# zyt334/AdaFace

Measured on AMD Instinct MI355X. Metric: 512x512 images/sec @ 50 DDIM steps, batch 8, higher is better.
Workload: dtype bf16

## Files before the change

adaface_amd/csrc/af_conv_gemm.hip:

```cpp
#include "af_kernels.h"

#include <cstdlib>
#include <cstring>
#include <mutex>
#include <type_traits>

template <int BM, int BN> struct TileCfg {
  static constexpr int XR = BM / 32, WR = BN / 32;
  static constexpr int WM = BM / 2, WN = BN / 2;
  static constexpr int MI = WM / 32, NI = WN / 32;
  static constexpr int TILE_BYTES = (BM + BN) * 128;
  static constexpr int EPI_LD = BN + 4;
  static constexpr int EPI_BYTES = BM * EPI_LD * 4;
  static constexpr int LDS_BYTES = (2 * TILE_BYTES > EPI_BYTES) ? 2 * TILE_BYTES : EPI_BYTES;
};

__device__ __forceinline__ void lds_dma16(__amdgpu_buffer_rsrc_t rs, char* lds_base, unsigned voffset, unsigned soffset) {
#if defined(__HIP_DEVICE_COMPILE__)
  __builtin_amdgcn_raw_ptr_buffer_load_lds(rs, (__attribute__((address_space(3))) void*)lds_base, 16, voffset, soffset,
                                           0, 0);
#endif
}

__device__ __forceinline__ void tile_coords(int wg, int nwg, int ntm, int ntn, int gm, int& tm, int& tn) {
// ... 525 lines not shown
        if (mok && (lane >> 4) == 0)
          *reinterpret_cast<float2*>(p.ln_stats_out + ((long)(tn * 2 + g) * p.M + m) * 2) = float2{ps, pq};
        continue;
      }
      if (slab) {
        if (m >= p.M) continue;
#pragma unroll
        for (int i = 0; i < NI; ++i) {
          if (i >= nblk) continue;
          *reinterpret_cast<f32x4*>(slab + (long)m * p.N + cbase + i * 16) = acc[i][j];
        }
        continue;
      }
      const bool mok2 = m < p.M;
      Quad<T> rq[NI], bq[NI];
      if (rowb && mok2) {
        const T* rp = rowb + (long)(p.howo_shift >= 0 ? m >> p.howo_shift : m / HoWo) * p.ldrb + cbase;
#pragma unroll
        for (int i = 0; i < NI; ++i) if (i < nblk) bq[i].load(rp + i * 16);
      }
      if (res && mok2) {
        const T* rp = res + (long)m * p.ldr + cbase;
#pragma unroll
        for (int i = 0; i < NI; ++i) if (i < nblk) rq[i].load(rp + i * 16);
      }
#pragma unroll
      for (int i = 0; i < NI; ++i) {
        if (i >= nblk) continue;
        Quad<T> o;
#pragma unroll
        for (int e = 0; e < 4; ++e) {
          float v = acc[i][j][e];
          if (rowb && mok2) v += to_f32<T>(bq[i].e[e]);
          if (res && mok2) v += to_f32<T>(rq[i].e[e]);
          o.e[e] = from_f32<T>(v);
        }
        wput(j, i, o);
      }
    }
    if (!slab) wflush();
    if (p.gn_stats_out && !slab && !geglu) {
      const int mslab = m0 + wq * 64;
      if (mslab < p.M) {
        float s = 0.f, q = 0.f;
        if (lane < HNo / 2) {
#pragma unroll 8
          for (int r = 0; r < 64; ++r) {
            const unsigned w = *reinterpret_cast<const unsigned*>(wtile + r * wpitch + lane * 4);
            const float a = __uint_as_float(w << 16), b = __uint_as_float(w & 0xffff0000u);
            s += a + b;
            q += a * a + b * b;
          }
        }
        float2* scr = reinterpret_cast<float2*>(wtile);
        scr[lane] = float2{s, q};
        const int hpg = p.gn_cpg >> 1, ng = (HNo / 2) / hpg;
        if (lane < ng) {
          float a = 0.f, b = 0.f;
          for (int t = 0; t < hpg; ++t) {
            const float2 v = scr[lane * hpg + t];
            a += v.x;
            b += v.y;
          }
          const int hw = 1 << p.howo_shift;
          const long part = ((long)(mslab >> p.howo_shift) * (hw >> 6) + ((mslab & (hw - 1)) >> 6)) * 32 + (ncol0 + g * HNo) / p.gn_cpg + lane;
          *reinterpret_cast<float2*>(p.gn_stats_out + part * 2) = float2{a, b};
        }
      }
    }
    return;
  }
  constexpr int ITEMS = BN / 32;
  const int nitems = geglu ? ITEMS / 2 : ITEMS;
#pragma unroll 1
  for (int pass = 0; pass < 2; ++pass) {
    if (pass) __syncthreads();
    if ((wq >> 1) == pass) {
      const int rbase = (wq & 1) * 64 + (lane & 15);
      const int nblk = geglu ? NI / 2 : NI;
#pragma unroll
      for (int j = 0; j < MI; ++j)
#pragma unroll
        for (int i = 0; i < NI; ++i)
          if (i < nblk)
            *reinterpret_cast<f32x4*>(et + (rbase + j * 16) * C::EPI_LD + g * HNo + i * 16 + cl) = acc[i][j];
    }
    __syncthreads();
    float v[ITEMS][8];
    int im[ITEMS], in_[ITEMS];
    Quad<T> rq[ITEMS][2], bq[ITEMS][2];
#pragma unroll
    for (int it = 0; it < ITEMS; ++it) {
      const int idx = tid + it * 512;
      const int row = geglu ? idx / (BN / 16) : idx / (BN / 8);
      const int c8 = (idx - row * tpr) * 8;
      const int m = m0 + pass * 128 + row, n = ncol0 + c8;
      const bool ok = it < nitems && m < p.M && n < Nvalid;
      im[it] = ok ? m : -1;
      in_[it] = n;
      if (!ok) continue;
      const float4 a = *reinterpret_cast<const float4*>(et + row * C::EPI_LD + c8);
      const float4 b4 = *reinterpret_cast<const float4*>(et + row * C::EPI_LD + c8 + 4);
      v[it][0] = a.x; v[it][1] = a.y; v[it][2] = a.z; v[it][3] = a.w;
      v[it][4] = b4.x; v[it][5] = b4.y; v[it][6] = b4.z; v[it][7] = b4.w;
      if (slab) continue;
      if (rowb) {
        const T* rp = rowb + (long)(p.howo_shift >= 0 ? m >> p.howo_shift : m / HoWo) * p.ldrb + n;
        bq[it][0].load(rp);
        bq[it][1].load(rp + 4);
      }
      if (res) {
        const T* rp = res + (long)m * p.ldr + n;
        rq[it][0].load(rp);
        rq[it][1].load(rp + 4);
      }
    }
#pragma unroll
    for (int it = 0; it < ITEMS; ++it) {
      const int m = im[it], n = in_[it];
      if (m < 0) continue;
      if (slab) {
        *reinterpret_cast<float4*>(slab + (long)m * p.N + n) = float4{v[it][0], v[it][1], v[it][2], v[it][3]};
        *reinterpret_cast<float4*>(slab + (long)m * p.N + n + 4) = float4{v[it][4], v[it][5], v[it][6], v[it][7]};
        continue;
      }
#pragma unroll
      for (int hq = 0; hq < 2; ++hq) {
        float* vv = v[it] + 4 * hq;
        if (rowb) {
#pragma unroll
          for (int e = 0; e < 4; ++e) vv[e] += to_f32<T>(bq[it][hq].e[e]);
        }
        if (res) {
#pragma unroll
          for (int e = 0; e < 4; ++e) vv[e] += to_f32<T>(rq[it][hq].e[e]);
        }
        Quad<T> o;
#pragma unroll
        for (int e = 0; e < 4; ++e) o.e[e] = from_f32<T>(vv[e]);
        o.store(out + (long)m * p.ldo + n + 4 * hq);
      }
    }
  }
}

template <int N> __device__ __forceinline__ void pp_wait_lgkm() {
  __builtin_amdgcn_sched_barrier(0);
  asm volatile("s_waitcnt lgkmcnt(%0)" ::"n"(N) : "memory");
  __builtin_amdgcn_sched_barrier(0);
}
typedef __attribute__((ext_vector_type(8))) int pp_i32x8;
typedef __attribute__((ext_vector_type(4))) int pp_i32x4;

template <int BN, bool GATHER, int LNMODE = 0, bool FP8 = false, int SCHED = FP8 ? 2 : 0>
__global__ __launch_bounds__(512) void conv_gemm_pp_kernel(const ConvGemmParams p) {
  constexpr bool NS = SCHED >= 1, MG = SCHED == 2;
  static_assert(MG || !FP8, "fp8 operands exist on the merged schedule only");
  using C = PpCfg<BN>;
  typedef bf16 T;
  static_assert(!FP8 || LNMODE == 0, "fp8 operands: plain epilogue only");
  constexpr unsigned XE = FP8 ? 1u : 2u;
  constexpr int NI = C::NI, MI = C::MI, SLOT = C::SLOT, XBYTES = C::XBYTES;
  constexpr int XP0 = MG ? C::XP / 2 : C::XP0;
  constexpr int NX0 = XP0 / 4, NX1 = (C::XP - XP0) / 4;
  constexpr int WP0 = MG ? (C::WP / 8) * 4 : 0;
  constexpr int NW0 = WP0 / 4, NW1 = (C::WP - WP0) / 4;
  constexpr int NP0 = NX0 + NW0, NP1 = NX1 + NW1, NPMAX = NP0 > NP1 ? NP0 : NP1;
  constexpr int NXM = NX0 > NX1 ? NX0 : NX1, NWM = NW0 > NW1 ? NW0 : NW1;
  static_assert(XP0 % 4 == 0 && WP0 % 4 == 0 && NW1 >= 1, "piece split");
  extern __shared__ __attribute__((aligned(1024))) char smem[];

  const int tid = threadIdx.x, lane = tid & 63, wid = __builtin_amdgcn_readfirstlane(tid >> 6);
  const int g = wid >> 2, wq = wid & 3;
  const int ntm = (p.M + 255) / 256, ntn = p.N / BN;
  int tm, tn;
  tile_coords(blockIdx.x, gridDim.x, ntm, ntn, p.group_m, tm, tn);
  const int m0 = tm * 256, n0 = tn * BN;
  const int zk = blockIdx.z;
  const int ph4 = (GATHER && p.phase4) ? (int)blockIdx.y : 0;
  const int pad_y = (GATHER && p.phase4) ? 1 - (ph4 >> 1) : p.pad, pad_x = (GATHER && p.phase4) ? 1 - (ph4 & 1) : p.pad;

  const __amdgpu_buffer_rsrc_t rs_x = __builtin_amdgcn_make_buffer_rsrc(
      const_cast<T*>(reinterpret_cast<const T*>(p.src)), 0, (int)0xFFFFFFF0u, 0x00020000);
  const __amdgpu_buffer_rsrc_t rs_w = __builtin_amdgcn_make_buffer_rsrc(
      const_cast<T*>(reinterpret_cast<const T*>(p.W)), 0, (int)0xFFFFFFF0u, 0x00020000);

  const int KT_all = p.K / (FP8 ? 128 : 64);
  const int kt_per = (KT_all + p.splitk - 1) / p.splitk;
  const int kt_begin = zk * kt_per;
  const int KT = min(KT_all, kt_begin + kt_per) - kt_begin;

  const int srow = lane >> 3;
  const unsigned dchunk = (unsigned)((lane & 7) ^ srow);
  const unsigned lchunk = (FP8 ? (dchunk & 3u) : dchunk) * 16u;
  const int HoWo = p.Ho * p.Wo;
  const unsigned ldcb = (unsigned)p.ldc * XE;
  const bool fast_taps = GATHER && ((p.up == 0 && p.ks * p.ks <= 31 && (p.fast_taps & 1)) || MG);
  unsigned x_off[NXM];
  int x_yx[GATHER ? NXM : 1];
  pp_static_for<0, NXM>([&](auto qc) {
    constexpr int q = decltype(qc)::value;
    const int piece = g == 0 ? wq + 4 * q : XP0 + wq + 4 * q;
    const int m = m0 + piece * 8 + srow;
    const bool ok = m < p.M && (g == 0 ? q < NX0 : q < NX1);
    const int mm = ok ? m : 0;
    int b, oy, ox;
    if (p.howo_shift >= 0 && p.wo_shift >= 0) {
      b = mm >> p.howo_shift;
      const int rem = mm & (HoWo - 1);
      oy = rem >> p.wo_shift;
      ox = rem & (p.Wo - 1);
    } else {
      b = mm / HoWo;
      const int rem = mm - b * HoWo;
      oy = rem / p.Wo;
      ox = rem - oy * p.Wo;
    }
    unsigned off = (unsigned)((long)b * p.src_batch_stride * XE) + lchunk;
    if constexpr (GATHER) {
      const int y0 = oy * p.stride - pad_y, x0 = ox * p.stride - pad_x;
      if (fast_taps) {
        int vy = 0, vx = 0;
        for (int k = 0; k < p.ks; ++k) {
          vy |= ((unsigned)(y0 + k) < (unsigned)p.Hi ? 1 : 0) << (k * p.ks);
          vx |= ((unsigned)(x0 + k) < (unsigned)p.Wi ? 1 : 0) << k;
        }
        int msk = 0;
        for (int k = 0; k < p.ks; ++k) msk |= ((vy >> (k * p.ks)) & 1) ? (vx << (k * p.ks)) : 0;
        x_yx[q] = ok ? msk : 0;
        off += (unsigned)(y0 * p.Ws + x0) * ldcb;
      } else {
        x_yx[q] = ok ? ((y0 << 16) | (x0 & 0xffff)) : (int)0xC0000000;
      }
    } else {
      off += (unsigned)(((oy * p.stride) >> p.up) * p.Ws + ((ox * p.stride) >> p.up)) * ldcb;
      if (!ok) off = 0xFFFFFFFFu;
    }
    x_off[q] = off;
  });
  unsigned w_off[NWM];
#pragma unroll
  for (int q = 0; q < NWM; ++q) {
    const int n = n0 + ((g == 0 ? 0 : WP0) + wq + 4 * q) * 8 + srow;
    w_off[q] = n < p.Wrows ? (unsigned)(((long)ph4 * p.Wrows + n) * p.ldw * XE) + dchunk * 16u : 0xFFFFFFFFu;
  }
  struct KWalk {
    int ky, kx, c0, ktile;
    int u_tap, u_c0;
  };
  KWalk kw;
  kw.ktile = kt_begin;
  kw.u_tap = 0; kw.u_c0 = 0;
  if (p.k_tap_inner) {
    const int taps = p.ks * p.ks;
    const int cc = kt_begin / taps, tap = kt_begin - cc * taps;
    kw.c0 = cc * 64;
    kw.ky = tap / p.ks;
    kw.kx = tap - kw.ky * p.ks;
  } else {
    const int k0 = kt_begin * 64;
    const int tap = k0 / p.Cin;
    kw.c0 = k0 - tap * p.Cin;
    kw.ky = tap / p.ks;
    kw.kx = tap - kw.ky * p.ks;
  }
  const int taps8 = p.ks * p.ks;
  const int adv_q = 2 / taps8, adv_r = 2 - adv_q * taps8;
  if constexpr (FP8) {
    const int u = 2 * kt_begin + (int)(dchunk >> 2);
    const int cc = u / taps8;
    kw.u_tap = u - cc * taps8;
    kw.u_c0 = cc * 64;
  }
  struct StageCtx {
    unsigned c0b, k0b;
    int live;
    int tapbit;
    unsigned delta;
    int u_ok;
    unsigned u_delta;
    int ky, kx, u_tap, u_c0;
  };
  auto x_addr = [&](auto qc, auto ftc, const StageCtx& sc) -> unsigned {
    constexpr int q = decltype(qc)::value;
    constexpr bool FT = decltype(ftc)::value;
    if constexpr (FP8) {
      if constexpr (GATHER) {
        if constexpr (FT) return ((x_yx[q] >> sc.u_tap) & sc.u_ok) ? x_off[q] + sc.u_delta : 0xFFFFFFFFu;
        const int kyl = p.ks == 3 ? (sc.u_tap * 11) >> 5 : 0, kxl = p.ks == 3 ? sc.u_tap - 3 * kyl : 0;
        const int iy = (x_yx[q] >> 16) + kyl, ix = ((x_yx[q] << 16) >> 16) + kxl;
        const bool ok = (unsigned)iy < (unsigned)p.Hi && (unsigned)ix < (unsigned)p.Wi && sc.u_c0 < p.Cin;
        const unsigned pix = (unsigned)((iy >> p.up) * p.Ws + (ix >> p.up));
        return ok ? x_off[q] + pix * ldcb + (unsigned)sc.u_c0 : 0xFFFFFFFFu;
      } else {
        return (sc.u_c0 < p.Cin && x_off[q] != 0xFFFFFFFFu) ? x_off[q] + (unsigned)sc.u_c0 : 0xFFFFFFFFu;
      }
    } else if constexpr (GATHER) {
      if constexpr (FT) return (x_yx[q] & sc.tapbit) ? x_off[q] + sc.delta : 0xFFFFFFFFu;
      const int iy = (x_yx[q] >> 16) + sc.ky, ix = ((x_yx[q] << 16) >> 16) + sc.kx;
      const bool ok = (unsigned)iy < (unsigned)p.Hi && (unsigned)ix < (unsigned)p.Wi;
      const unsigned pix = (unsigned)((iy >> p.up) * p.Ws + (ix >> p.up));
      return ok ? x_off[q] + pix * ldcb : 0xFFFFFFFFu;
    } else {
      return x_off[q];
    }
  };
  auto stage_begin = [&](const KWalk& k) -> StageCtx {
    StageCtx sc;
    sc.tapbit = 0; sc.delta = 0u; sc.u_ok = 0; sc.u_delta = 0u;
    sc.ky = k.ky; sc.kx = k.kx; sc.u_tap = k.u_tap; sc.u_c0 = k.u_c0;
// ... 62 lines not shown
  auto wait_keep1 = [&]() { if (g == 0) pp_wait_vm<NP0>(); else pp_wait_vm<NP1>(); };

  const unsigned lds0 = (unsigned)(__UINTPTR_TYPE__)((__attribute__((address_space(3))) char*)smem);
  const unsigned fch0 = (unsigned)((lane >> 4) ^ (lane & 7)) * 16u;
  const unsigned fch1 = (unsigned)(((lane >> 4) + 4) ^ (lane & 7)) * 16u;
  const unsigned x_base = (unsigned)((wq * 64 + (lane & 15)) * 128);
  const unsigned w_base = (unsigned)(XBYTES + (g * C::HN + (lane & 15)) * 128);

  f32x4 acc[NI][MI];
#pragma unroll
  for (int i = 0; i < NI; ++i)
#pragma unroll
    for (int j = 0; j < MI; ++j) acc[i][j] = f32x4{0.f, 0.f, 0.f, 0.f};
  pp_u32x4 xf[MI][2], wf[NI][2];
#pragma unroll
  for (int i = 0; i < NI; ++i) wf[i][1] = pp_u32x4{0u, 0u, 0u, 0u};
#pragma unroll
  for (int j = 0; j < MI; ++j) xf[j][1] = pp_u32x4{0u, 0u, 0u, 0u};

  auto half = [&](int slot_off, auto rc, auto mc) {
    constexpr int ur = decltype(rc)::value, um = decltype(mc)::value;
    const unsigned b = lds0 + (unsigned)slot_off + (ur ? fch1 : fch0);
    pp_static_for<0, NI * MI>([&](auto nc) {
      constexpr int n = decltype(nc)::value;
      constexpr int i = n / MI, j = n % MI;
      if constexpr (n < NI) wf[n][ur] = pp_lds_read128<n * 2048>(b + w_base);
      else if constexpr (n < NI + MI) xf[n - NI][ur] = pp_lds_read128<(n - NI) * 2048>(b + x_base);
      acc[i][j] = __builtin_amdgcn_mfma_f32_16x16x32_bf16(__builtin_bit_cast(bf16x8, wf[i][um]),
                                                          __builtin_bit_cast(bf16x8, xf[j][um]), acc[i][j], 0, 0, 0);
      if constexpr (n < NI + MI) __builtin_amdgcn_sched_barrier(0);
    });
  };
  std::integral_constant<int, 0> U0;
  std::integral_constant<int, 1> U1;

  const int cl = 4 * (lane >> 4);
  float4 bias_r[NI];
  auto load_bias = [&]() {
#pragma unroll
    for (int i = 0; i < NI; ++i) {
      bias_r[i] = float4{0.f, 0.f, 0.f, 0.f};
      if (p.bias && p.splitk <= 1) bias_r[i] = *reinterpret_cast<const float4*>(p.bias + n0 + g * C::HN + i * 16 + cl);
    }
  };
  if constexpr (!NS) load_bias();

  float4 ln_cs[LNMODE == 1 ? NI : 1];
  float ln_mu[LNMODE == 1 ? MI : 1], ln_rs[LNMODE == 1 ? MI : 1];
  if constexpr (LNMODE == 1) {
#pragma unroll
    for (int i = 0; i < NI; ++i) ln_cs[i] = *reinterpret_cast<const float4*>(p.ln_colsum + n0 + g * C::HN + i * 16 + cl);
#pragma unroll
    for (int j = 0; j < MI; ++j) {
      const int m = m0 + wq * 64 + j * 16 + (lane & 15);
      float2 st = float2{0.f, 0.f};
      if (m < p.M) st = *reinterpret_cast<const float2*>(p.ln_stats + (long)m * 2);
      ln_mu[j] = st.x;
      ln_rs[j] = st.y;
    }
  }

  pp_u32x4 w8[NS ? NI : 1][2], xa8[NS ? MI : 1][2], xb8[NS ? MI : 1][2];
  int wsc8[FP8 ? NI : 1];
  int xsc8 = p.x_scale_e8;
  if constexpr (NS && !FP8) {
#pragma unroll
    for (int i = 0; i < NI; ++i) w8[i][0] = w8[i][1] = pp_u32x4{0u, 0u, 0u, 0u};
#pragma unroll
    for (int j = 0; j < MI; ++j) xa8[j][0] = xa8[j][1] = xb8[j][0] = xb8[j][1] = pp_u32x4{0u, 0u, 0u, 0u};
  }
  if constexpr (FP8) {
    asm volatile("" : "+v"(xsc8));
#pragma unroll
    for (int i = 0; i < NI; ++i) {
      w8[i][0] = w8[i][1] = pp_u32x4{0u, 0u, 0u, 0u};
      wsc8[i] = (int)p.w_scale[n0 + g * C::HN + i * 16 + (lane & 15)];
    }
#pragma unroll
    for (int j = 0; j < MI; ++j) xa8[j][0] = xa8[j][1] = xb8[j][0] = xb8[j][1] = pp_u32x4{0u, 0u, 0u, 0u};
  }
  auto mfma8 = [&](f32x4& c, const pp_u32x4 (&wv)[2], const pp_u32x4 (&xv)[2], int wscale) {
    if constexpr (!FP8) {
      c = __builtin_amdgcn_mfma_f32_16x16x32_bf16(__builtin_bit_cast(bf16x8, wv[0]), __builtin_bit_cast(bf16x8, xv[0]), c, 0, 0, 0);
      c = __builtin_amdgcn_mfma_f32_16x16x32_bf16(__builtin_bit_cast(bf16x8, wv[1]), __builtin_bit_cast(bf16x8, xv[1]), c, 0, 0, 0);
      asm volatile("" : "+v"(c));
      return;
    }
    const pp_i32x8 a = __builtin_shufflevector(__builtin_bit_cast(pp_i32x4, wv[0]), __builtin_bit_cast(pp_i32x4, wv[1]), 0, 1, 2, 3, 4, 5, 6, 7);
    const pp_i32x8 b = __builtin_shufflevector(__builtin_bit_cast(pp_i32x4, xv[0]), __builtin_bit_cast(pp_i32x4, xv[1]), 0, 1, 2, 3, 4, 5, 6, 7);
    c = __builtin_amdgcn_mfma_scale_f32_16x16x128_f8f6f4(a, b, c, 0, 0, 0, wscale, 0, xsc8);
    asm volatile("" : "+v"(c));
  };
  auto wait_block = [&](auto nc, pp_u32x4 (&blk)[2]) {
    constexpr int n = decltype(nc)::value;
    asm volatile("s_waitcnt lgkmcnt(%2)" : "+v"(blk[0]), "+v"(blk[1]) : "n"(n) : "memory");
  };
#ifdef AF_LAB_ABLATE
  const int lab = p.fast_taps >> 4;
#else
  constexpr int lab = 0;
#endif
  auto cphase8 = [&](int slot_off, pp_u32x4 (&xc)[NS ? MI : 1][2], pp_u32x4 (&xp)[NS ? MI : 1][2], auto ftc, int stage_off,
                     const StageCtx& sc) {
    if constexpr (NS) {
      constexpr int NB = NI + MI;
      char* sbase = smem + stage_off;
      const unsigned b0 = lds0 + (unsigned)slot_off + fch0, b1 = lds0 + (unsigned)slot_off + fch1;
      auto rd_block = [&](auto bc) {
        constexpr int bi = decltype(bc)::value;
        if (lab & 2) return;
        if constexpr (bi == 0) {
          w8[0][0] = pp_lds_read128<0>(b0 + w_base);
          w8[0][1] = pp_lds_read128<0>(b1 + w_base);
        } else if constexpr (bi <= MI) {
          xc[bi - 1][0] = pp_lds_read128<(bi - 1) * 2048>(b0 + x_base);
          xc[bi - 1][1] = pp_lds_read128<(bi - 1) * 2048>(b1 + x_base);
        } else {
          w8[bi - MI][0] = pp_lds_read128<(bi - MI) * 2048>(b0 + w_base);
          w8[bi - MI][1] = pp_lds_read128<(bi - MI) * 2048>(b1 + w_base);
        }
      };
      rd_block(std::integral_constant<int, 0>{});
      rd_block(std::integral_constant<int, 1>{});
      __builtin_amdgcn_sched_barrier(0);
      pp_static_for<0, MI * NI>([&](auto mc) {
        constexpr int m = decltype(mc)::value;
        if constexpr (m < MI) {
          if (!(lab & 4)) mfma8(acc[NI - 1][m], w8[NI - 1], xp[m], wsc8[FP8 ? NI - 1 : 0]);
        } else {
          constexpr int i = (m - MI) / MI, j = (m - MI) % MI;
          constexpr int issued = (2 + m) < NB ? (2 + m) : NB;
          constexpr int need = i == 0 ? 1 + j : (j == 0 ? MI + i : -1);
          if constexpr (need >= 0) {
            std::integral_constant<int, 2 * (issued - need - 1)> cnt;
            if constexpr (i == 0) wait_block(cnt, xc[j]); else wait_block(cnt, w8[i]);
            if constexpr (i == 0 && j == 0) wait_block(cnt, w8[0]);
          }
          if (!(lab & 4)) mfma8(acc[i][j], w8[i], xc[j], wsc8[FP8 ? i : 0]);
        }
        if constexpr (2 + m < NB) rd_block(std::integral_constant<int, 2 + m>{});
        if constexpr (MG && m >= MI && (m - MI) / 2 < NPMAX) {
          if (!(lab & 1) && (g == ((m - MI) & 1) || !p.pp_stagger)) {
            if (p.pp_stagger || ((m - MI) & 1) == 0) stage_piece(std::integral_constant<int, (m - MI) / 2>{}, ftc, sbase, sc);
          }
        }
        __builtin_amdgcn_sched_barrier(0);
      });
      static_assert(!MG || MI + 2 * (NPMAX - 1) + 1 < MI * NI, "merged schedule: a staging slot behind an MFMA for every piece");
      pp_wait_lgkm0();
    }
  };

  int rd = 0, w0 = SLOT, w1 = 2 * SLOT;
  if constexpr (MG) {
    stage(0);
    stage(SLOT);
    auto tile = [&](auto& xc, auto& xp) {
      if (g == 0) pp_wait_vm<NP0>(); else pp_wait_vm<NP1>();
      __builtin_amdgcn_s_barrier();
      const StageCtx sc = stage_begin(kw);
      cphase8(rd, xc, xp, std::integral_constant<bool, GATHER>{}, w1, sc);
      kw = kw_next(kw);
      const int tmp = rd; rd = w0; w0 = w1; w1 = tmp;
    };
    for (int t = 0; t + 1 < KT; t += 2) {
      tile(xa8, xb8);
      tile(xb8, xa8);
    }
    if (KT & 1) tile(xa8, xb8);
    pp_wait_vm<0>();
    if (KT & 1) {
#pragma unroll
      for (int j = 0; j < MI; ++j) mfma8(acc[NI - 1][j], w8[NI - 1], xa8[j], wsc8[FP8 ? NI - 1 : 0]);
    } else {
#pragma unroll
      for (int j = 0; j < MI; ++j) mfma8(acc[NI - 1][j], w8[NI - 1], xb8[j], wsc8[FP8 ? NI - 1 : 0]);
    }
    __builtin_amdgcn_s_barrier();
  }
  if constexpr (!MG) {
  stage(0);
  if (g == 1) {
    if (KT > 1) { stage(SLOT); wait_keep1(); } else pp_wait_vm<0>();
  }
  __builtin_amdgcn_s_barrier();
  if (g == 1) __builtin_amdgcn_s_barrier();
  }
  auto dphase = [&](int t) {
    if (g == 0) {
      if (t + 1 < KT) { stage(w0); wait_keep1(); } else pp_wait_vm<0>();
    } else {
      if (t + 2 < KT) stage(w1);
    }
    __builtin_amdgcn_s_barrier();
  };
  auto cend = [&](int t) {
    if (g == 1) { if (t + 2 < KT) wait_keep1(); else pp_wait_vm<0>(); }
    __builtin_amdgcn_s_barrier();
    const int tmp = rd; rd = w0; w0 = w1; w1 = tmp;
  };
  if constexpr (MG) {
  } else if constexpr (NS) {
    auto tile1 = [&](int t, auto& xc, auto& xp) {
      dphase(t);
      __builtin_amdgcn_s_setprio(1);
      cphase8(rd, xc, xp, std::false_type{}, 0, StageCtx{});
      __builtin_amdgcn_s_setprio(0);
      cend(t);
    };
    int t = 0;
    for (; t + 1 < KT; t += 2) {
      tile1(t, xa8, xb8);
      tile1(t + 1, xb8, xa8);
    }
    if (KT & 1) tile1(t, xa8, xb8);
    if (KT & 1) {
#pragma unroll
      for (int j = 0; j < MI; ++j) mfma8(acc[NI - 1][j], w8[NI - 1], xa8[j], wsc8[FP8 ? NI - 1 : 0]);
    } else {
#pragma unroll
      for (int j = 0; j < MI; ++j) mfma8(acc[NI - 1][j], w8[NI - 1], xb8[j], wsc8[FP8 ? NI - 1 : 0]);
    }
  } else {
    for (int t = 0; t < KT; ++t) {
      dphase(t);
      __builtin_amdgcn_s_setprio(1);
      half(rd, U0, U1);
      pp_wait_lgkm0();
      half(rd, U1, U0);
      pp_wait_lgkm0();
      __builtin_amdgcn_s_setprio(0);
      cend(t);
    }
#pragma unroll
    for (int i = 0; i < NI; ++i)
#pragma unroll
      for (int j = 0; j < MI; ++j)
        acc[i][j] = __builtin_amdgcn_mfma_f32_16x16x32_bf16(__builtin_bit_cast(bf16x8, wf[i][1]),
                                                            __builtin_bit_cast(bf16x8, xf[j][1]), acc[i][j], 0, 0, 0);
  }
  if constexpr (!MG) { if (g == 0) __builtin_amdgcn_s_barrier(); }
  if constexpr (NS) load_bias();

  pp_epilogue<BN, LNMODE>(p, acc, bias_r, ln_cs, ln_mu, ln_rs, smem, tid, lane, g, wq, m0, n0, tn, zk);
}

#ifdef AF_LAB_ABLATE
__device__ unsigned long long g_lab_stamps[2048 * 5];
extern "C" int af_lab_stamps(unsigned long long* out, int n) {
  return hipMemcpyFromSymbol(out, HIP_SYMBOL(g_lab_stamps), sizeof(unsigned long long) * (size_t)n) == hipSuccess ? 0 : -1;
}
__device__ __forceinline__ unsigned long long lab_now() {
  unsigned long long t;
  __builtin_amdgcn_sched_barrier(0);
  asm volatile("s_memrealtime %0\n\ts_waitcnt lgkmcnt(0)" : "=s"(t)::"memory");
  __builtin_amdgcn_sched_barrier(0);
  return t;
}
#endif
struct Halo8Cfg {
  static constexpr int BN = 160;
  static constexpr int HPIX = 400, HBUF = HPIX * 128, WBYTES = BN * 128;
  static constexpr int W_BASE = 2 * HBUF, LDS_BYTES = 2 * HBUF + 3 * WBYTES;
  static constexpr int NHQ = 7;
  static_assert(LDS_BYTES <= 160 * 1024, "LDS budget");
};

template <int LABL>
__global__ __launch_bounds__(512) void conv3x3_halo8_kernel(const ConvGemmParams p) {
  using C = PpCfg<160>;
  using H = Halo8Cfg;
  typedef bf16 T;
  constexpr int BN = 160, NI = C::NI, MI = C::MI, NHQ = H::NHQ;
  extern __shared__ __attribute__((aligned(1024))) char smem[];
  const int tid = threadIdx.x, lane = tid & 63, wid = __builtin_amdgcn_readfirstlane(tid >> 6);
  const int g = wid >> 2, wq = wid & 3;
  const int ntm = p.M / 256, ntn = p.N / BN;
  int tm, tn;
  tile_coords(blockIdx.x, gridDim.x, ntm, ntn, p.group_m, tm, tn);
  const int m0 = tm * 256, n0 = tn * BN;
  const int zk = blockIdx.z;
  T* const xsrc = const_cast<T*>(reinterpret_cast<const T*>(p.src));
  T* const wsrc = const_cast<T*>(reinterpret_cast<const T*>(p.W));
  const __amdgpu_buffer_rsrc_t rs_x = __builtin_amdgcn_make_buffer_rsrc(xsrc, 0, (int)0xFFFFFFF0u, 0x00020000);
  const __amdgpu_buffer_rsrc_t rs_w = __builtin_amdgcn_make_buffer_rsrc(wsrc, 0, (int)0xFFFFFFF0u, 0x00020000);

  const int KT_all = p.K / 64;
  const int kt_per = (KT_all + p.splitk - 1) / p.splitk;
  const int kt_begin = zk * kt_per;
#ifdef AF_LAB_ABLATE
  const int lab = p.fast_taps >> 4;
  const int KT = (lab & 16) ? 9 : min(KT_all, kt_begin + kt_per) - kt_begin;
#else
  constexpr int lab = 0;
  const int KT = min(KT_all, kt_begin + kt_per) - kt_begin;
#endif
  const int chunk0 = kt_begin / 9;
  const int nch = KT / 9;
#ifdef AF_LAB_ABLATE
  unsigned long long st0 = 0, st1 = 0, st2 = 0;
  if (lab & 64) st0 = lab_now();
#endif

  const int Wo = p.Wo, HW = Wo + 2, wsh = p.wo_shift;
  const int R = 256 >> wsh;
  const int HP = (R + 2) * HW;
  const int img = m0 >> p.howo_shift;
// ... 1203 lines not shown
  const long nbs = nb * s;
  const double fill = (double)nbs / (double)(((nbs + 255) / 256) * 256);
  if (fill < g_af_knobs.gemm_pp_minfill * 0.01) return pl;
  pl.tile = cand;
  pl.splitk = s;
  if (s > 1) pl.ws_bytes = (size_t)s * p.M * p.N * sizeof(float);
  plan_group_m(pl, p);
  return pl;
}

AfGemmPlan af_plan_conv_gemm(const ConvGemmParams& p, int batch, int elem_size) {
  if (p.fp8) return plan_fp8(p, batch);
  AfGemmPlan pl;
  pl.tile = 0;
  pl.splitk = 1;
  pl.ws_bytes = 0;
  const bool geglu = p.epilogue == AF_EPI_GEGLU;
  const bool n128 = geglu || (p.N % 128) == 0 || p.N > 640;
  static const int bm[4] = {128, 64, 128, 64}, bn[4] = {128, 128, 64, 64};
  static const double eff[4] = {1.0, 0.88, 0.88, 0.72};
  double best = 1e30;
  for (int t = 0; t < 4; ++t) {
    if (n128 && bn[t] != 128) continue;
    if (!n128 && bn[t] != 64) continue;
    const long nb = (long)((p.M + bm[t] - 1) / bm[t]) * ((p.N + bn[t] - 1) / bn[t]) * batch;
    const double rounds = (double)((nb + 255) / 256);
    const double cost = rounds * bm[t] * bn[t] / eff[t];
    if (cost < best) { best = cost; pl.tile = t; }
  }
  const int BK = 128 / elem_size;
  const int KT = p.K / BK;
  const long nb = (long)((p.M + bm[pl.tile] - 1) / bm[pl.tile]) * ((p.N + bn[pl.tile] - 1) / bn[pl.tile]) * batch;
  if (batch == 1 && !geglu && nb < 256 && KT >= 16) {
    const int target = g_af_knobs.splitk_target;
    int s = (int)((target + nb - 1) / nb);
    if (s > KT / 8) s = KT / 8;
    if (s > 16) s = 16;
    if (s >= 2) {
      pl.tile = n128 ? 0 : 2;
      const long nb2 = (long)((p.M + bm[pl.tile] - 1) / bm[pl.tile]) * ((p.N + bn[pl.tile] - 1) / bn[pl.tile]);
      s = (int)((target + nb2 - 1) / nb2);
      if (s > KT / 8) s = KT / 8;
      if (s > 16) s = 16;
      if (s >= 2) pl.splitk = s;
    }
  }
  if (g_af_knobs.small_m_tile64 && batch == 1 && !geglu && p.M <= 1024 && p.N % 64 == 0 && KT <= 32) {
    const long nb64 = (long)((p.M + 63) / 64) * (p.N / 64);
    if (nb64 >= 64 && nb64 <= 1024) { pl.tile = 3; pl.splitk = 1; }
  }
  pl.halo_tw = 0;
  if (p.ks == 3 && p.stride == 1 && p.up == 0 && p.pad == 1 && batch == 1 && !geglu && pl.splitk == 1 &&
      p.Ho == p.Hi && p.Wo == p.Wi && p.ldc >= p.Cin && g_af_knobs.conv_halo) {
    if (p.Wo % 32 == 0 && p.Ho % 4 == 0) pl.halo_tw = 32;
    else if (p.Wo % 16 == 0 && p.Ho % 8 == 0) pl.halo_tw = 16;
    if (pl.halo_tw) {
      const long nb128 = (long)(p.M / 128) * ((p.N + 127) / 128), nb64 = (long)(p.M / 128) * ((p.N + 63) / 64);
      const double c128 = (double)((nb128 + 255) / 256) * 128, c64 = (double)((nb64 + 255) / 256) * 64 / 0.9;
      pl.tile = (n128 && c128 <= c64) ? 0 : 2;
      if (!n128 && (p.N % 64) != 0) pl.tile = 2;
    }
  }
  if (elem_size == 2 && batch == 1 && p.K % 64 == 0 && p.Cin % 64 == 0 && g_af_knobs.gemm_pp) {
    int cand = -1;
    if (!geglu && p.N % 160 == 0) cand = 5;
    else if (p.N % 128 == 0) cand = 4;
    if (cand >= 0) {
      const int tbn = cand == 5 ? 160 : 128;
      const long nb = (long)((p.M + 255) / 256) * (p.N / tbn);
      int s = 1;
      if (!geglu && nb < 208) {
        s = (int)((256 + nb / 2) / nb);
        if (s > KT / 16) s = KT / 16;
        if (s > 16) s = 16;
        if (s < 1) s = 1;
      }
      const long nbs = nb * s;
      const double fill = (double)nbs / (double)(((nbs + 255) / 256) * 256);
      if (fill >= g_af_knobs.gemm_pp_minfill * 0.01 && p.M >= 512) {
        pl.tile = cand;
        pl.splitk = s;
        pl.halo_tw = 0;
      }
    }
  }
  if (pl.tile == 5 && pl.halo_tw == 0 && p.ks == 3 && p.stride == 1 && p.pad == 1 && p.up == 0 && p.Ho == p.Hi && p.Wo == p.Wi &&
      (p.Wo == 16 || p.Wo == 32 || p.Wo == 64) && (p.Ho & (p.Ho - 1)) == 0 && p.Ho >= 256 / p.Wo && p.M % 256 == 0 &&
      p.K == 9 * p.Cin && p.ldc >= p.Cin && (g_af_knobs.conv_halo8 & 1) && !p.ln_stats && !p.ln_stats_out) {
    pl.halo_tw = 256;
    while (pl.splitk > 1 && (p.Cin / 64) % pl.splitk != 0) --pl.splitk;
  }
  if (elem_size == 2 && (g_af_knobs.conv_halo8 & 2) && g_af_knobs.gemm_pp && af_conv_s8_ok(p, batch) && !p.gn_stats_out &&
      (p.Wo <= 16 || (g_af_knobs.conv_halo8 & 4))) {
    pl.tile = 5;
    pl.halo_tw = 8;
    pl.splitk = af_conv_s8_slices(p, batch);
  }
  const int ft = g_af_knobs.gemm_tile;
  if (ft >= 0 && ft < 4 && !(geglu && bn[ft] != 128)) pl.tile = ft;
  const int fs = g_af_knobs.gemm_splitk;
  if (fs >= 1 && batch == 1 && !geglu) pl.splitk = fs > KT ? KT : fs;
  if (pl.halo_tw == 8 && (pl.tile != 5 || pl.splitk != af_conv_s8_slices(p, batch))) pl.halo_tw = 0;
  if (pl.splitk > 1 && pl.halo_tw != 256 && pl.halo_tw != 8) pl.halo_tw = 0;
  if (pl.halo_tw == 256 && (pl.tile != 5 || (p.Cin / 64) % pl.splitk != 0)) pl.halo_tw = 0;
  if (pl.splitk > 1) pl.ws_bytes = (size_t)pl.splitk * p.M * p.N * sizeof(float);
  plan_group_m(pl, p);
  return pl;
}

static void plan_group_m(AfGemmPlan& pl, const ConvGemmParams& p) {
  static const int bm[4] = {128, 64, 128, 64}, bn[4] = {128, 128, 64, 64};
  {
    const bool h4 = pl.halo_tw != 0 && pl.halo_tw != 256 && pl.halo_tw != 8;
    const int tbm = h4 ? 128 : (pl.tile >= 4 ? 256 : bm[pl.tile]);
    const int tbn = h4 ? ((pl.tile == 0 || pl.tile == 1) ? 128 : 64) : (pl.tile == 5 ? 160 : pl.tile == 4 ? 128 : bn[pl.tile]);
    const int MT = (p.M + tbm - 1) / tbm, NT = (p.N + tbn - 1) / tbn;
    const int resident = pl.tile >= 4 ? 32 : 32 * ((tbm * tbn >= 128 * 128) ? 2 : 3);
    const bool taps_reuse = pl.halo_tw || (pl.tile >= 4 && p.ks > 1 && (g_af_knobs.conv_tap_inner || p.fp8));
    const double xb = (double)p.M * (p.K / (p.ks * p.ks)) * (taps_reuse ? (p.stride == 1 ? 1.5 : 1.0) : (double)(p.ks * p.ks) / (p.stride * p.stride));
    const double wb = (double)p.N * p.K;
    double bestc = 1e300;
    int bestg = 1;
    for (int gmm = 1; gmm <= 64; gmm *= 2) {
      const int gm_eff = gmm < MT ? gmm : MT;
      int gn_eff = resident / gm_eff;
      if (gn_eff < 1) gn_eff = 1;
      if (gn_eff > NT) gn_eff = NT;
      const double c = xb * ((double)NT / gn_eff) + wb * ((double)MT / gm_eff);
      if (c < bestc * 0.999) { bestc = c; bestg = gmm; }
    }
    pl.group_m = g_af_knobs.gemm_groupm >= 1 ? g_af_knobs.gemm_groupm : bestg;
  }
}

template <typename T, int BM, int BN, bool DMA>
static int launch_cfg2(const ConvGemmParams& p, int batch, hipStream_t stream) {
  using C = TileCfg<BM, BN>;
  static unsigned long long attr_done = 0;
  if (int rc = af_ensure_dynamic_lds(attr_done, reinterpret_cast<const void*>(&conv_gemm_kernel<T, BM, BN, DMA>), C::LDS_BYTES)) return rc;
  const int ntm = (p.M + BM - 1) / BM, ntn = (p.N + BN - 1) / BN;
  dim3 grid(ntm * ntn, 1, p.splitk > 1 ? p.splitk : batch);
  hipLaunchKernelGGL((conv_gemm_kernel<T, BM, BN, DMA>), grid, dim3(256), C::LDS_BYTES, stream, p);
  HIP_CHECK_RET(hipGetLastError());
  return 0;
}
template <typename T, int BM, int BN>
static int launch_cfg(const ConvGemmParams& p, int batch, hipStream_t stream) {
  const int force = g_af_knobs.gemm_dma;
  const int kt_per_slice = p.K / (128 / (int)sizeof(T)) / (p.splitk > 1 ? p.splitk : 1);
  const bool use_dma = force >= 0 ? force != 0 : kt_per_slice >= 32;
  return use_dma ? launch_cfg2<T, BM, BN, true>(p, batch, stream) : launch_cfg2<T, BM, BN, false>(p, batch, stream);
}

template <int BN, int LNMODE, bool GATHER, bool FP8, int SCHED>
static int launch_pp_one(const ConvGemmParams& p, dim3 grid, hipStream_t stream) {
  using C = PpCfg<BN>;
  static unsigned long long attr_done = 0;
  if (int rc = af_ensure_dynamic_lds(attr_done, reinterpret_cast<const void*>(&conv_gemm_pp_kernel<BN, GATHER, LNMODE, FP8, SCHED>), C::LDS_BYTES)) return rc;
  hipLaunchKernelGGL((conv_gemm_pp_kernel<BN, GATHER, LNMODE, FP8, SCHED>), grid, dim3(512), C::LDS_BYTES, stream, p);
  HIP_CHECK_RET(hipGetLastError());
  return 0;
}
template <int BN, int LNMODE, bool GATHER> static int launch_pp_sched(const ConvGemmParams& p, dim3 grid, hipStream_t stream) {
  int sched = g_af_knobs.pp_sched;
  if (sched >= 2 && GATHER && !(p.up == 0 && p.ks * p.ks <= 31)) sched = 1;
  if (p.epilogue == AF_EPI_GEGLU && g_af_knobs.pp_sched == 2) sched = 0;
  switch (sched) {
    case 0: return launch_pp_one<BN, LNMODE, GATHER, false, 0>(p, grid, stream);
    case 1: return launch_pp_one<BN, LNMODE, GATHER, false, 1>(p, grid, stream);
    default: return launch_pp_one<BN, LNMODE, GATHER, false, 2>(p, grid, stream);
  }
}
template <int BN> static int launch_pp(const ConvGemmParams& p, hipStream_t stream) {
  const bool gather = !(p.ks == 1 && p.pad == 0);
  dim3 grid(((p.M + 255) / 256) * (p.N / BN), 1, p.splitk > 1 ? p.splitk : 1);
  if (p.ln_stats || p.ln_stats_out) {
    if (gather || p.splitk > 1 || (p.ln_stats && p.ln_stats_out) || (p.ln_stats_out && p.epilogue == AF_EPI_GEGLU)) {
      af_set_error_msg("conv_gemm: LayerNorm-fused launch needs a 1x1 GEMM without split-K");
      return -1;
    }
    return p.ln_stats ? launch_pp_sched<BN, 1, false>(p, grid, stream) : launch_pp_sched<BN, 2, false>(p, grid, stream);
  }
  return gather ? launch_pp_sched<BN, 0, true>(p, grid, stream) : launch_pp_sched<BN, 0, false>(p, grid, stream);
}

template <int BN> static int launch_pp8(const ConvGemmParams& p, hipStream_t stream) {
  const bool gather = !(p.ks == 1 && p.pad == 0);
  dim3 grid(((p.M + 255) / 256) * (p.N / BN), 1, p.splitk > 1 ? p.splitk : 1);
  return gather ? launch_pp_one<BN, 0, true, true, 2>(p, grid, stream) : launch_pp_one<BN, 0, false, true, 2>(p, grid, stream);
}

static int launch_conv_gemm_fp8(ConvGemmParams p, hipStream_t stream, const AfGemmPlan* plan, void* ws) {
  if (p.K % 128 != 0 || p.Cin % 64 != 0 || (p.ks != 1 && p.ks != 3) || p.K < p.ks * p.ks * p.Cin || p.ldw < p.K ||
      p.ldw % 16 != 0 || p.ldc % 16 != 0 || p.ldc < p.Cin || !p.w_scale || p.epilogue == AF_EPI_GEGLU || p.ln_stats || p.ln_stats_out) {
    af_set_error_msg("conv_gemm fp8: K=%d Cin=%d ks=%d ldw=%d ldc=%d (need K%%128==0, Cin%%64==0, ks 1|3, 16-byte pitches, row scales)",
                     p.K, p.Cin, p.ks, p.ldw, p.ldc);
    return -1;
  }
  if (p.N % 4 != 0 || p.ldo % 4 != 0 || (p.residual && p.ldr % 4 != 0) || (p.rowbias && p.ldrb % 4 != 0)) {
    af_set_error_msg("conv_gemm fp8: N/ldo/ldr/ldrb must be multiples of 4 (N=%d ldo=%d)", p.N, p.ldo);
    return -1;
  }
  if (p.M <= 0 || p.N <= 0) return 0;
  {
    const int HoWo = p.Ho * p.Wo > 0 ? p.Ho * p.Wo : 1;
    const double nb = (double)((p.M + HoWo - 1) / HoWo);
    if (nb * (double)p.src_batch_stride >= 4294967280.0 || (double)p.Wrows * p.ldw >= 4294967280.0) {
      af_set_error_msg("conv_gemm fp8: operand exceeds the 4 GB range of the 32-bit gather offsets (split the batch)");
      return -1;
    }
  }
  AfGemmPlan pl = plan ? *plan : af_plan_conv_gemm(p, 1, 2);
  if (pl.tile != 4 && pl.tile != 5) {
    af_set_error_msg("conv_gemm fp8: shape M=%d N=%d K=%d has no fp8 plan (ask af_plan_conv_gemm first)", p.M, p.N, p.K);
    return -1;
  }
  if (pl.splitk > 1 && !ws) pl.splitk = 1;
  p.splitk = pl.splitk;
  p.ws = ws;
  af_set_last_plan(pl);
  g_af_plan_counts[10] += 1;
  if (pl.splitk > 1) g_af_plan_counts[7] += 1;
  {
    auto lg2 = [](int v) { int s = 0; while ((1 << s) < v) ++s; return (v > 0 && (1 << s) == v) ? s : -1; };
    p.howo_shift = lg2(p.Ho * p.Wo);
    p.wo_shift = lg2(p.Wo);
  }
  p.group_m = pl.group_m > 0 ? pl.group_m : 1;
  p.pp_epilogue = g_af_knobs.pp_direct < 0 ? 0 : (g_af_knobs.pp_direct ? 2 : 1);
  if (p.gn_stats_out) {
    if (!af_conv_gn_stats_ok(p, pl, p.gn_cpg)) {
      af_set_error_msg("conv_gemm fp8: GroupNorm partial sums asked of a launch that cannot write them");
      return -1;
    }
    p.pp_epilogue = 2;
    g_af_plan_counts[14] += 1;
  }
  p.k_tap_inner = 1;
  p.fast_taps = g_af_knobs.conv_fast_taps;
  p.pp_stagger = g_af_knobs.pp_stagger;
  AfProfScope prof(AF_K_PP_FP8, stream, 2.0 * p.M * (double)p.N * (p.k_logical ? p.k_logical : p.K),
                   (double)p.M * p.Cin + (double)p.N * p.K + (double)p.M * p.N * 2.0);
  const int rc = pl.tile == 4 ? launch_pp8<128>(p, stream) : launch_pp8<160>(p, stream);
  if (rc) return rc;
  if (p.splitk > 1) {
    const long nq = (long)p.M * (p.N >> 2);
    unsigned blocks = (unsigned)((nq + 255) / 256);
    if (blocks > 4096) blocks = 4096;
    hipLaunchKernelGGL((splitk_reduce_kernel<bf16>), dim3(blocks), dim3(256), 0, stream, p);
    HIP_CHECK_RET(hipGetLastError());
  }
  return 0;
}

template <int LABL> static int launch_halo8_lab(const ConvGemmParams& p, hipStream_t stream) {
  static unsigned long long attr_done = 0;
  if (int rc = af_ensure_dynamic_lds(attr_done, reinterpret_cast<const void*>(&conv3x3_halo8_kernel<LABL>), Halo8Cfg::LDS_BYTES))
    return rc;
  dim3 grid((p.M / 256) * (p.N / 160), 1, p.splitk > 1 ? p.splitk : 1);
  hipLaunchKernelGGL(conv3x3_halo8_kernel<LABL>, grid, dim3(512), Halo8Cfg::LDS_BYTES, stream, p);
  HIP_CHECK_RET(hipGetLastError());
  return 0;
}
static int launch_halo8(const ConvGemmParams& p, hipStream_t stream) {
  if (p.Cin % 64 != 0 || (p.Cin / 64) % (p.splitk > 1 ? p.splitk : 1) != 0) {
    af_set_error_msg("conv_gemm: halo kernel needs K slices of whole 64-channel chunks (Cin=%d splitk=%d)", p.Cin, p.splitk);
    return -1;
  }
#ifdef AF_LAB_ABLATE
  switch ((p.fast_taps >> 4) & 7) {
    case 1: return launch_halo8_lab<1>(p, stream);
    case 2: return launch_halo8_lab<2>(p, stream);
    case 3: return launch_halo8_lab<3>(p, stream);
    case 4: return launch_halo8_lab<4>(p, stream);
    case 5: return launch_halo8_lab<5>(p, stream);
    case 6: return launch_halo8_lab<6>(p, stream);
    case 7: return launch_halo8_lab<7>(p, stream);
    default: break;
  }
#endif
  return launch_halo8_lab<0>(p, stream);
}

template <typename T, int TW, int BN> static int launch_halo(const ConvGemmParams& p, hipStream_t stream) {
  using C = HaloCfg<TW, BN>;
  static unsigned long long attr_done = 0;
  if (int rc = af_ensure_dynamic_lds(attr_done, reinterpret_cast<const void*>(&conv3x3_halo_kernel<T, TW, BN>), C::LDS_BYTES)) return rc;
  dim3 grid((p.M / 128) * ((p.N + BN - 1) / BN), 1, 1);
  hipLaunchKernelGGL((conv3x3_halo_kernel<T, TW, BN>), grid, dim3(256), C::LDS_BYTES, stream, p);
  HIP_CHECK_RET(hipGetLastError());
  return 0;
}

__global__ __launch_bounds__(256) void up_phase4_weights_kernel(const bf16* __restrict__ w3, bf16* __restrict__ w4, long total,
                                                                int rows, int cin, int ldw3) {
  const long idx = (long)blockIdx.x * 256 + threadIdx.x;
  if (idx >= total) return;
  const int n = (int)(idx / cin), c = (int)(idx - (long)n * cin);
  float w[3][3];
#pragma unroll
  for (int ky = 0; ky < 3; ++ky)
#pragma unroll
    for (int kx = 0; kx < 3; ++kx) w[ky][kx] = to_f32<bf16>(w3[(long)n * ldw3 + (ky * 3 + kx) * cin + c]);
  const long ld4 = 4L * cin;
#pragma unroll
  for (int ph = 0; ph < 4; ++ph) {
    const int dy = ph >> 1, dx = ph & 1;
#pragma unroll
    for (int ty = 0; ty < 2; ++ty)
#pragma unroll
      for (int tx = 0; tx < 2; ++tx) {
        const int ylo = ty == 0 ? 0 : (dy == 0 ? 1 : 2), yhi = ty == 0 ? (dy == 0 ? 0 : 1) : 2;
        const int xlo = tx == 0 ? 0 : (dx == 0 ? 1 : 2), xhi = tx == 0 ? (dx == 0 ? 0 : 1) : 2;
        float sum = 0.f;
#pragma unroll
        for (int ky = 0; ky < 3; ++ky)
#pragma unroll
          for (int kx = 0; kx < 3; ++kx)
            if (ky >= ylo && ky <= yhi && kx >= xlo && kx <= xhi) sum += w[ky][kx];
        w4[((long)ph * rows + n) * ld4 + (ty * 2 + tx) * cin + c] = from_f32<bf16>(sum);
      }
  }
}
// ... 265 lines not shown
```

Before: 10.83.

## Add compile-time unrolled K walk for 3x3 gather conv GEMM merged schedule

Adds a CTW variant of the ping-pong conv GEMM kernel that fully unrolls the K loop over the 3x3 taps, so the LDS ring slot, tap index, kx/ky offsets and staging pieces become compile-time constants per position. Out-of-range gather addresses are masked with a precomputed per-piece bit mask rather than runtime address logic. The intent is to cut scalar and vector address arithmetic and runtime branching inside the merged MFMA/DMA schedule. It only applies to staggered, non-split-K 3x3 convolutions with tap-inner K ordering. Code size grows and the tail handling gets more complex. Ablation variants are compiled only under a lab macro.

New measurement: 10.85 (median of 6 runs). Within noise of the previous version (+0.1%).

```diff
diff --git a/adaface_amd/csrc/af_conv_gemm.hip b/adaface_amd/csrc/af_conv_gemm.hip
--- a/adaface_amd/csrc/af_conv_gemm.hip
+++ b/adaface_amd/csrc/af_conv_gemm.hip
@@ -701,10 +701,12 @@
 typedef __attribute__((ext_vector_type(8))) int pp_i32x8;
 typedef __attribute__((ext_vector_type(4))) int pp_i32x4;
 
-template <int BN, bool GATHER, int LNMODE = 0, bool FP8 = false, int SCHED = FP8 ? 2 : 0>
+template <int BN, bool GATHER, int LNMODE = 0, bool FP8 = false, int SCHED = FP8 ? 2 : 0, bool CTW = false, int LABL = 0>
 __global__ __launch_bounds__(512) void conv_gemm_pp_kernel(const ConvGemmParams p) {
   constexpr bool NS = SCHED >= 1, MG = SCHED == 2;
   static_assert(MG || !FP8, "fp8 operands exist on the merged schedule only");
+  static_assert(!CTW || (MG && !FP8 && LNMODE == 0), "compile-time K walk: bf16 merged schedule, plain epilogue");
+  static_assert(CTW || LABL == 0, "lab bits of the compile-time walk");
   using C = PpCfg<BN>;
   typedef bf16 T;
   static_assert(!FP8 || LNMODE == 0, "fp8 operands: plain epilogue only");
@@ -1073,7 +1075,152 @@
   };
 
   int rd = 0, w0 = SLOT, w1 = 2 * SLOT;
-  if constexpr (MG) {
+  if constexpr (CTW) {
+    const unsigned xr0 = lds0 + x_base + fch0, xr1 = lds0 + x_base + fch1;
+    const unsigned wr0 = lds0 + w_base + fch0, wr1 = lds0 + w_base + fch1;
+    unsigned xbad[GATHER ? NXM : 1];
+#pragma unroll
+    for (int q = 0; q < (GATHER ? NXM : 1); ++q) {
+      if constexpr (GATHER) {
+        xbad[q] = ~(unsigned)x_yx[q];
+#ifdef AF_LAB_ABLATE
+        if (p.fast_taps & 0x100) xbad[q] |= ~1u;
+#endif
+      } else {
+        xbad[q] = 0u;
+      }
+    }
+    const unsigned cin2 = (unsigned)p.Cin * 2u, rowp = (unsigned)p.Ws * ldcb;
+    auto dma = [&](__amdgpu_buffer_rsrc_t rs, char* dst, unsigned voff, unsigned soff) {
+      if constexpr ((LABL & 1) == 0) lds_dma16(rs, dst, voff, soff);
+    };
+    auto mfma2 = [&](f32x4& c, const pp_u32x4 (&wv)[2], const pp_u32x4 (&xv)[2]) {
+      if constexpr ((LABL & 4) == 0) mfma8(c, wv, xv, 0);
+    };
+    auto wait_block2 = [&](auto nc, pp_u32x4 (&b0)[2], pp_u32x4 (&b1)[2]) {
+      constexpr int n = decltype(nc)::value;
+      asm volatile("s_waitcnt lgkmcnt(%4)" : "+v"(b0[0]), "+v"(b0[1]), "+v"(b1[0]), "+v"(b1[1]) : "n"(n) : "memory");
+    };
+    auto step = [&](auto gc, auto rsc, pp_u32x4 (&xp)[MI][2], unsigned xs2, unsigned ks2, int t2, unsigned dx2, int live2) {
+      constexpr int G = decltype(gc)::value, RS = decltype(rsc)::value;
+      constexpr int SS = (RS + 2) % 3, NB = NI + MI;
+      constexpr int NXG = G == 0 ? NX0 : NX1, NPG = G == 0 ? NP0 : NP1, XPB = G == 0 ? 0 : XP0, WPB = G == 0 ? 0 : WP0;
+      pp_wait_vm<NPG>();
+      __builtin_amdgcn_s_barrier();
+      unsigned dead2 = live2 ? 0u : 0xFFFFFFFFu;
+      if (!__builtin_constant_p(live2)) asm("" : "+v"(dead2));
+      const unsigned bx0 = xr0 + RS * SLOT, bx1 = xr1 + RS * SLOT, bw0 = wr0 + RS * SLOT, bw1 = wr1 + RS * SLOT;
+      char* const sdst = smem + SS * SLOT + wq * 1024;
+      pp_u32x4 xc[MI][2];
+      if constexpr ((LABL & 2) != 0) {
+#pragma unroll
+        for (int j = 0; j < MI; ++j) xc[j][0] = xc[j][1] = pp_u32x4{0u, 0u, 0u, 0u};
+      }
+      auto rd_block = [&](auto bc) {
+        constexpr int bi = decltype(bc)::value;
+        if constexpr ((LABL & 2) != 0) {
+        } else if constexpr (bi == 0) {
+          w8[0][0] = pp_lds_read128<0>(bw0);
+          w8[0][1] = pp_lds_read128<0>(bw1);
+        } else if constexpr (bi <= MI) {
+          xc[bi - 1][0] = pp_lds_read128<(bi - 1) * 2048>(bx0);
+          xc[bi - 1][1] = pp_lds_read128<(bi - 1) * 2048>(bx1);
+        } else {
+          w8[bi - MI][0] = pp_lds_read128<(bi - MI) * 2048>(bw0);
+          w8[bi - MI][1] = pp_lds_read128<(bi - MI) * 2048>(bw1);
+        }
+      };
+      auto stage_q = [&](auto qc) {
+        constexpr int q = decltype(qc)::value;
+        if constexpr (q < NXG) {
+          unsigned a = x_off[q];
+          if constexpr (GATHER) {
+            unsigned bad;
+            asm("v_bfe_i32 %0, %1, %2, 1" : "=v"(bad) : "v"(xbad[q]), "s"(t2));
+            a = (a + dx2) | bad;
+          }
+          dma(rs_x, sdst + (XPB + 4 * q) * 1024, a | dead2, xs2);
+        } else if constexpr (q < NPG) {
+          dma(rs_w, sdst + XBYTES + (WPB + 4 * (q - NXG)) * 1024, w_off[q - NXG] | dead2, ks2);
+        }
+      };
+      rd_block(std::integral_constant<int, 0>{});
+      rd_block(std::integral_constant<int, 1>{});
+      __builtin_amdgcn_sched_barrier(0);
+      pp_static_for<0, MI * NI>([&](auto mc) {
+        constexpr int m = decltype(mc)::value;
+        if constexpr (m < MI) {
+          mfma2(acc[NI - 1][m], w8[NI - 1], xp[m]);
+        } else {
+          constexpr int i = (m - MI) / MI, j = (m - MI) % MI;
+          constexpr int issued = (2 + m) < NB ? (2 + m) : NB;
+          constexpr int need = i == 0 ? 1 + j : (j == 0 ? MI + i : -1);
+          if constexpr (need >= 0) {
+            std::integral_constant<int, 2 * (issued - need - 1)> cnt;
+            if constexpr (i == 0 && j == 0) wait_block2(cnt, xc[0], w8[0]);
+            else if constexpr (i == 0) wait_block(cnt, xc[j]);
+            else wait_block(cnt, w8[i]);
+          }
+          mfma2(acc[i][j], w8[i], xc[j]);
+        }
+        if constexpr (2 + m < NB) rd_block(std::integral_constant<int, 2 + m>{});
+        if constexpr (m >= MI && ((m - MI) & 1) == G && (m - MI) / 2 < NPG) stage_q(std::integral_constant<int, (m - MI) / 2>{});
+        __builtin_amdgcn_sched_barrier(0);
+      });
+      static_assert(MI + 2 * (NPMAX - 1) + 1 < MI * NI, "merged schedule: a staging slot behind an MFMA for every piece");
+      pp_wait_lgkm0();
+#pragma unroll
+      for (int j = 0; j < MI; ++j) xp[j][0] = xc[j][0], xp[j][1] = xc[j][1];
+    };
+    using std::integral_constant;
+    constexpr int B = GATHER ? 9 : 6;
+    stage(0);
+    stage(SLOT);
+    const int tap0 = GATHER ? kt_begin % 9 : 0;
+    auto walk = [&](auto gc) {
+      pp_u32x4 xp[MI][2];
+#pragma unroll
+      for (int j = 0; j < MI; ++j) xp[j][0] = xp[j][1] = pp_u32x4{0u, 0u, 0u, 0u};
+      unsigned xs = GATHER ? (unsigned)(kt_begin / 9) * 128u : (unsigned)kt_begin * 128u;
+      auto pos = [&](auto pc, int live2) {
+        constexpr int P = decltype(pc)::value;
+        if constexpr (GATHER) {
+          const int u = tap0 + (P + 2);
+          const int cy = u >= 18 ? 2 : (u >= 9 ? 1 : 0);
+          const int t2 = u - 9 * cy, ky = (t2 * 11) >> 5, kx = t2 - 3 * ky;
+          const unsigned xs2 = xs + (unsigned)cy * 128u;
+          step(gc, integral_constant<int, P % 3>{}, xp, xs2, (unsigned)t2 * cin2 + xs2, t2, (unsigned)ky * rowp + (unsigned)kx * ldcb,
+               live2);
+        } else {
+          const unsigned k2 = xs + (P + 2) * 128u;
+          step(gc, integral_constant<int, P % 3>{}, xp, k2, k2, 0, 0u, live2);
+        }
+      };
+      int n = KT;
+      for (; n > B; n -= B, xs += (GATHER ? 1u : (unsigned)B) * 128u)
+        pp_static_for<0, B>([&](auto pc) { pos(pc, decltype(pc)::value < B - 1 ? 1 : (n > B + 1 ? 1 : 0)); });
+      if (n > 0) {
+        do {
+          pos(integral_constant<int, 0>{}, n > 2); if (n <= 1) break;
+          pos(integral_constant<int, 1>{}, n > 3); if (n <= 2) break;
+          pos(integral_constant<int, 2>{}, n > 4); if (n <= 3) break;
+          pos(integral_constant<int, 3>{}, n > 5); if (n <= 4) break;
+          pos(integral_constant<int, 4>{}, n > 6); if (n <= 5) break;
+          pos(integral_constant<int, 5>{}, n > 7); if (n <= 6) break;
+          if constexpr (GATHER) {
+            pos(integral_constant<int, 6>{}, n > 8); if (n <= 7) break;
+            pos(integral_constant<int, 7>{}, 0); if (n <= 8) break;
+            pos(integral_constant<int, 8>{}, 0);
+          }
+        } while (0);
+      }
+      pp_wait_vm<0>();
+#pragma unroll
+      for (int j = 0; j < MI; ++j) mfma2(acc[NI - 1][j], w8[NI - 1], xp[j]);
+    };
+    if (g == 0) walk(integral_constant<int, 0>{}); else walk(integral_constant<int, 1>{});
+    __builtin_amdgcn_s_barrier();
+  } else if constexpr (MG) {
     stage(0);
     stage(SLOT);
     auto tile = [&](auto& xc, auto& xp) {
@@ -2583,14 +2730,29 @@
   return use_dma ? launch_cfg2<T, BM, BN, true>(p, batch, stream) : launch_cfg2<T, BM, BN, false>(p, batch, stream);
 }
 
-template <int BN, int LNMODE, bool GATHER, bool FP8, int SCHED>
+template <int BN, int LNMODE, bool GATHER, bool FP8, int SCHED, bool CTW = false, int LABL = 0>
 static int launch_pp_one(const ConvGemmParams& p, dim3 grid, hipStream_t stream) {
   using C = PpCfg<BN>;
   static unsigned long long attr_done = 0;
-  if (int rc = af_ensure_dynamic_lds(attr_done, reinterpret_cast<const void*>(&conv_gemm_pp_kernel<BN, GATHER, LNMODE, FP8, SCHED>), C::LDS_BYTES)) return rc;
-  hipLaunchKernelGGL((conv_gemm_pp_kernel<BN, GATHER, LNMODE, FP8, SCHED>), grid, dim3(512), C::LDS_BYTES, stream, p);
+  if (int rc = af_ensure_dynamic_lds(attr_done, reinterpret_cast<const void*>(&conv_gemm_pp_kernel<BN, GATHER, LNMODE, FP8, SCHED, CTW, LABL>), C::LDS_BYTES)) return rc;
+  hipLaunchKernelGGL((conv_gemm_pp_kernel<BN, GATHER, LNMODE, FP8, SCHED, CTW, LABL>), grid, dim3(512), C::LDS_BYTES, stream, p);
   HIP_CHECK_RET(hipGetLastError());
   return 0;
+}
+template <int BN, bool GATHER> static int launch_pp_ctw(const ConvGemmParams& p, dim3 grid, hipStream_t stream) {
+#ifdef AF_LAB_ABLATE
+  switch ((p.fast_taps >> 4) & 7) {
+    case 1: return launch_pp_one<BN, 0, GATHER, false, 2, true, 1>(p, grid, stream);
+    case 2: return launch_pp_one<BN, 0, GATHER, false, 2, true, 2>(p, grid, stream);
+    case 3: return launch_pp_one<BN, 0, GATHER, false, 2, true, 3>(p, grid, stream);
+    case 4: return launch_pp_one<BN, 0, GATHER, false, 2, true, 4>(p, grid, stream);
+    case 5: return launch_pp_one<BN, 0, GATHER, false, 2, true, 5>(p, grid, stream);
+    case 6: return launch_pp_one<BN, 0, GATHER, false, 2, true, 6>(p, grid, stream);
+    case 7: return launch_pp_one<BN, 0, GATHER, false, 2, true, 7>(p, grid, stream);
+    default: break;
+  }
+#endif
+  return launch_pp_one<BN, 0, GATHER, false, 2, true, 0>(p, grid, stream);
 }
 template <int BN, int LNMODE, bool GATHER> static int launch_pp_sched(const ConvGemmParams& p, dim3 grid, hipStream_t stream) {
   int sched = g_af_knobs.pp_sched;
@@ -2599,7 +2761,12 @@
   switch (sched) {
     case 0: return launch_pp_one<BN, LNMODE, GATHER, false, 0>(p, grid, stream);
     case 1: return launch_pp_one<BN, LNMODE, GATHER, false, 1>(p, grid, stream);
-    default: return launch_pp_one<BN, LNMODE, GATHER, false, 2>(p, grid, stream);
+    default:
+      if constexpr (LNMODE == 0 && GATHER) {
+        if (p.pp_stagger && p.splitk <= 1 && p.ks == 3 && p.k_tap_inner && !p.phase4 && p.K == 9 * p.Cin && p.Cin % 64 == 0)
+          return launch_pp_ctw<BN, GATHER>(p, grid, stream);
+      }
+      return launch_pp_one<BN, LNMODE, GATHER, false, 2>(p, grid, stream);
   }
 }
 template <int BN> static int launch_pp(const ConvGemmParams& p, hipStream_t stream) {
```
